# Mouafak-Khaled/Flow-Q-Learning

Hardware: AMD Instinct MI355X
Metric: FQL grad-steps/sec (whole node) over 16-α population, cube-single-v0 (higher is better)
Workload: dtype f32

## Files before the change

### flow-q-learning_amd/csrc/kernels.h

```cpp
#pragma once
#include <hip/hip_runtime.h>
#include <stdint.h>

namespace fq {

struct TRef {
    float* p;
    long long ss;
    long long sy;
};

inline TRef tref(float* p, long long ss, long long sy = 0) { return TRef{p, ss, sy}; }

enum GemmLayout { LAYOUT_FWD = 0, LAYOUT_DX = 1, LAYOUT_DW = 2 };
enum GemmEpi { EPI_STORE = 0, EPI_BIAS = 1, EPI_BIAS_GELU2 = 2, EPI_BIAS_GELU = 3, EPI_ADAM = 4 };

struct GemmArgs {
    TRef A, B, C, C2, bias;
    int M, N, K;
    int lda, ldb, ldc;
    int ny, nz;
    const int* slots;
    unsigned long long* probe;
};
// ... 87 lines not shown
};
void launch_head_fwd(int mode, const HeadArgs& a, hipStream_t s);

struct StreamArgs {
    const float* params;
    long long P, ens;
    long long w_off[EF_MAX_LAYERS + 1], b_off[EF_MAX_LAYERS + 1];
    long long g_off[EF_MAX_LAYERS], be_off[EF_MAX_LAYERS];
    const float* x0;
    long long x0_ss;
    int ld_x, K0, L, M;
    float* U[EF_MAX_LAYERS];
    float* G[EF_MAX_LAYERS];
    float* MU[EF_MAX_LAYERS];
    float* RS[EF_MAX_LAYERS];
    long long s_ss, s_sy, st_ss, st_sy;
    int ld_s, st_lo, st_hi;
    int g_hi;
    HeadArgs head;
    int ny, nz;
    const int* slots;
};
bool stream_fwd_supported(int H, int L, int K0, int nout, int M);
void launch_stream_fwd(int head_mode, bool ln, const StreamArgs& a, hipStream_t s);

struct SplitSync {
    unsigned long long* xch;
    unsigned* cnt;
    unsigned* gen;
    unsigned* err;
};
struct SplitFwdArgs {
    StreamArgs s;
    TRef aflow;
    int D, A, S, first;
    float steps_f;
    unsigned long long* probe;
    SplitSync sync;
    unsigned long long* phase;
    float* pre0;
};
long long split_cluster_bytes();
constexpr long long split_euler_pre0_floats() { return 2LL * 256 * 16; }
bool split_euler_pre0(int K0, int D);
int split_counter_stride();
bool split_fwd_supported(int H, int L, int K0, int nout, int M);
void launch_split_fwd(int head_mode, bool ln, bool euler, int F, const SplitFwdArgs& a, hipStream_t s);
// ... 273 lines not shown
```

### flow-q-learning_amd/csrc/kernels.hip

```cpp
#include "kernels.h"

#include <hip/hip_runtime.h>
#include <math.h>

#include <type_traits>

#if defined(__HIP_DEVICE_COMPILE__) && !defined(__gfx950__)
#error "fqlpop kernels target gfx950 (MI355X) only: the s_waitcnt immediates use the gfx9 encoding"
#endif


namespace fq {

typedef float f32x16 __attribute__((ext_vector_type(16)));
typedef float f32x4 __attribute__((ext_vector_type(4)));

#define DEV __device__ __forceinline__

DEV float* at(TRef t, int slot, int y = 0) {
    return t.p + (long long)slot * t.ss + (long long)y * t.sy;
}

constexpr float kSqrt2OverPi = 0.7978845608028654f;

// ... 161 lines not shown
        float* st = a.stats + ((long long)slot * a.n_total_chunks + ci) * 3;
        st[0] = mx;
        st[1] = mn;
        st[2] = ss;
    }
}
DEV void adam_chunk(const AdamArgs& a, int bx, int z) { adam_chunk_t<256>(a, bx, z); }



typedef __amdgpu_buffer_rsrc_t rsrc_t;
DEV rsrc_t make_rsrc(const float* p, long long n_elems) {
    return __builtin_amdgcn_make_buffer_rsrc((void*)p, (short)0, (int)(n_elems * 4), 0x00020000);
}
DEV float4 bload4(rsrc_t r, int elem_off) {
    return __builtin_bit_cast(float4, __builtin_amdgcn_raw_buffer_load_b128(r, elem_off * 4, 0, 0));
}
DEV float bload1(rsrc_t r, int voff_b, int soff_b) {
    return __builtin_bit_cast(float, __builtin_amdgcn_raw_buffer_load_b32(r, voff_b, soff_b, 0));
}
DEV void bstore1(rsrc_t r, float v, int voff_b, int soff_b) {
    __builtin_amdgcn_raw_buffer_store_b32(__builtin_bit_cast(int, v), r, voff_b, soff_b, 0);
}

template <int NT>
DEV void load_in0(float* in0, const float* x, int K0, int ld, int c0) {
    constexpr int N = 64 * 16 + 64, IT = (N + NT - 1) / NT;
    static_assert(N >= 16, "");
    const rsrc_t rX = make_rsrc(x, (long long)K0 * ld);
    float v[IT];
#pragma unroll
    for (int q = 0; q < IT; ++q) {
        const int e = min((int)threadIdx.x + q * NT, N - 1), r = e >> 4, j = e & 15;
        v[q] = bload1(rX, (r * ld + c0 + j) * 4, 0);
    }
#pragma unroll
    for (int q = 0; q < IT; ++q) {
        const int e = (int)threadIdx.x + q * NT;
        if (e < N) in0[e] = v[q];
    }
}

template <int TILE, int BK, bool RC>
DEV float4 stage_load(rsrc_t X, int ld, int p, int i0, int k0) {
    const int idx = threadIdx.x + 256 * p;
    if constexpr (RC) {
        const int row = idx / (BK / 4), c = (idx % (BK / 4)) * 4;
        return bload4(X, (i0 + row) * ld + k0 + c);
    } else {
        const int row = idx / (TILE / 4), c = (idx % (TILE / 4)) * 4;
        return bload4(X, (k0 + row) * ld + i0 + c);
    }
}

template <int BK, bool KB>
constexpr int rc_pitch() { return KB ? BK + 4 : BK + 1; }
// ... 1170 lines not shown
#pragma unroll
        for (int s = 0; s < 16; ++s) w5r[s] = li < nout ? w5r[s] : 0.f;
        f32x4 hacc = f32x4{0.f, 0.f, 0.f, 0.f};
#pragma unroll
        for (int s = 0; s < 16; ++s)
            hacc = __builtin_amdgcn_mfma_f32_16x16x4f32(w5r[s], slab[(64 * w + 4 * s + lk) * NC + li], hacc, 0, 0, 0);
        float* hred = in0;
        if (lk < 2) {
#pragma unroll
            for (int r = 0; r < 4; ++r) hred[w * 8 * NC + (4 * lk + r) * NC + li] = hacc[r];
        }
        __syncthreads();
        if (tid < nout * NC) {
            const int j = tid / NC, col = tid % NC;
            float v = hred[tid];
#pragma unroll
            for (int q = 1; q < EF_NW; ++q) v += hred[q * 8 * NC + tid];
            v += P[g.b_off[L] + j];
            head_write<MODE>(g.head, slot, y, j, c0 + col, v);
        }
    }
}

void launch_stream_fwd(int head_mode, bool ln, const StreamArgs& a, hipStream_t s) {
    const dim3 grid((a.M / EF_NC) * a.ny * a.nz), block(EF_NW * 64);
#define FQ_SF(MODE, LNV) hipLaunchKernelGGL((stream_fwd_kernel<MODE, LNV>), grid, block, 0, s, a)
    switch (head_mode) {
        case HEAD_BC_FUSED: if (ln) FQ_SF(HEAD_BC_FUSED, true); else FQ_SF(HEAD_BC_FUSED, false); break;
        case HEAD_OS: if (ln) FQ_SF(HEAD_OS, true); else FQ_SF(HEAD_OS, false); break;
        default: if (ln) FQ_SF(HEAD_STORE, true); else FQ_SF(HEAD_STORE, false); break;
    }
#undef FQ_SF
}

constexpr int SP_NW = 4, SP_NT = SP_NW * 64;
constexpr int SP_XG = EF_H * EF_NC;
constexpr int SP_G_HP = 2 * SP_XG;
constexpr int SP_G_LP = SP_G_HP + 8 * 8 * EF_NC;
constexpr int SP_G_N = SP_G_LP + 2 * 8 * 2 * EF_NC;
constexpr long long SP_CLUSTER_GRANULES = (SP_G_N + 31) / 32 * 32;
constexpr int SP_CNT_STRIDE = 16;
constexpr unsigned SP_SPIN_LIMIT = 1u << 21;

long long split_cluster_bytes() { return SP_CLUSTER_GRANULES * 8; }
int split_counter_stride() { return SP_CNT_STRIDE; }

typedef __attribute__((address_space(1))) unsigned int gu32_t;
typedef __attribute__((address_space(1))) unsigned long long gu64_t;

// ... 2708 lines not shown
```

### flow-q-learning_amd/csrc/runtime.cpp

```cpp
#include <hip/hip_runtime.h>

#include <algorithm>
#include <cmath>
#include <cstdio>
#include <cstdlib>
#include <cstring>
#include <functional>
#include <map>
#include <set>
#include <memory>
#include <string>
#include <vector>

#include "../../include/fqlpop.h"
#include "kernels.h"

using namespace fq;

namespace {

thread_local std::string g_err;

struct FqErr {
    int code;
// ... 16 lines not shown
long long align_up(long long x) { return (x + kAlign - 1) / kAlign * kAlign; }

#ifdef FQ_DIAG
const char* diag_env(const char* name) { return std::getenv(name); }
#else
const char* diag_env(const char*) { return nullptr; }
#endif

struct EngineOptions {
    int euler_fused = 1;
    int stream_fwd = 1;
    int stream_bwd = 1;
    int fused_adam = 1;
    int serial = 0;
    int dw_tile_critic = 10, dw_tile_actor = 10;
    int adam_nt = 3;
    int split = 1;
    int small_sched = 1;
    int split_blocks = 256;
    int split_sites = 0;
    int hw_queues = 4;
    int em_seq_sweep = 1;
    int em_ens_xcd = 0;
};
EngineOptions g_engine_opts;

constexpr int kStepBranches = 4;
int step_streams(const EngineOptions& eo) {
    return (eo.serial || eo.hw_queues < kStepBranches) ? 1 : kStepBranches;
}

struct EngineOptionRef {
    const char* name;
    int EngineOptions::*field;
    int lo, hi;
};
const EngineOptionRef kEngineOptions[] = {
    {"euler_fused", &EngineOptions::euler_fused, 0, 1}, {"stream_fwd", &EngineOptions::stream_fwd, 0, 1},
    {"stream_bwd", &EngineOptions::stream_bwd, 0, 1},   {"fused_adam", &EngineOptions::fused_adam, 0, 1},
    {"serial", &EngineOptions::serial, 0, 1},
    {"dw_tile_critic", &EngineOptions::dw_tile_critic, 0, 10},
    {"dw_tile_actor", &EngineOptions::dw_tile_actor, 0, 10},
    {"adam_nt", &EngineOptions::adam_nt, 0, 3},
    {"split", &EngineOptions::split, 0, 8},
    {"small_sched", &EngineOptions::small_sched, 0, 1},
    {"hw_queues", &EngineOptions::hw_queues, 1, 1024},
    {"split_sites", &EngineOptions::split_sites, 0, (1 << 24) - 1},
    {"split_blocks", &EngineOptions::split_blocks, 64, 1024},
    {"em_seq_sweep", &EngineOptions::em_seq_sweep, 0, 1},
    {"em_ens_xcd", &EngineOptions::em_ens_xcd, 0, 1},
};

void philox_host(uint32_t c[4], uint32_t k0, uint32_t k1) {
    for (int r = 0; r < 10; ++r) {
        const uint64_t p0 = (uint64_t)0xD2511F53u * c[0], p1 = (uint64_t)0xCD9E8D57u * c[2];
        const uint32_t hi0 = (uint32_t)(p0 >> 32), lo0 = (uint32_t)p0;
        const uint32_t hi1 = (uint32_t)(p1 >> 32), lo1 = (uint32_t)p1;
        const uint32_t n0 = hi1 ^ c[1] ^ k0, n2 = hi0 ^ c[3] ^ k1;
        c[0] = n0; c[1] = lo1; c[2] = n2; c[3] = lo0;
        k0 += 0x9E3779B9u;
        k1 += 0xBB67AE85u;
    }
}

uint64_t sample_key(uint64_t seed, float alpha) {
    uint32_t ab;
    std::memcpy(&ab, &alpha, sizeof(ab));
    uint64_t z = seed ^ ((uint64_t)ab << 32 | 0x9E3779B9u);
    z = (z ^ (z >> 30)) * 0xBF58476D1CE4E5B9ull;
    z = (z ^ (z >> 27)) * 0x94D049BB133111EBull;
    return z ^ (z >> 31);
}

// ... 54 lines not shown
    const Buf* X = nullptr;
    int ld = 0;
    int ld_d = 0, ld_o = 0;
    long long sy = 0, st_sy = 0;
    bool keep_u = true;
    bool dominant = false;
    std::vector<Buf> U, G, MU, RS, DU;
    Buf DH, C1, C2, part;
    int fwd_site = -1, bwd_site = -1;
    int skip_fwd = 0, skip_bwd = 0;
    TRef par(long long off) const { return tref(*arena + lay->off + off, arena_ss, lay->ens_size); }
    TRef act(const Buf& b, long long coff = 0) const { return b.cols(coff, sy); }
    TRef stat(const Buf& b, long long coff = 0) const { return b.cols(coff, st_sy); }
    TRef grad(const Buf& b) const { return b.ref((long long)lay->H * ld_d); }
};

}

struct fqlpop {
    fqlpop_config cfg{};
    EngineOptions opt{};
    int n = 0;
    int device = 0;
    int D = 0, A = 0, H = 0, L = 0, B = 0, E = 0, S = 0;
    NetLayout critic, bc, os;
    long long P = 0, PT = 0;
    std::vector<Leaf> leaves;
    long long state_size = 0;

    float* params_buf[2] = {nullptr, nullptr};
    Buf paramsT_buf[2];
    int cur = 0;
    float *params = nullptr, *params_nx = nullptr;
    float *grads = nullptr, *adam_m = nullptr, *adam_v = nullptr, *target = nullptr;
    int* count = nullptr;
    uint64_t* seeds = nullptr;
    uint64_t* skeys = nullptr;
    float* alpha = nullptr;
    int* slots = nullptr;
    float* stats = nullptr;
    Chunk* chunks = nullptr;
    int* chunk_leaf = nullptr;
    int* leaf_first = nullptr;
    int n_chunks_net[3] = {0, 0, 0}, chunk_base_net[3] = {0, 0, 0}, n_chunks_total = 0;
    bool fused_adam = false;
    int w_stat_base[3][EF_MAX_LAYERS] = {};
// ... 311 lines not shown
                                                                                        : kSplitMaxClusters;
}
constexpr long long kSplitMaxBlocks = 256;

int split_factor_opts(const EngineOptions& o, bool split_ok, int site, long long clusters, bool min4,
                      long long max_blocks) {
    int opt = o.split;
    const int code = (o.split_sites >> (3 * site)) & 7;
    if (code == 1) return 1;
    if (code >= 2 && code <= 4) {
        opt = 1 << (code - 1);
        max_blocks = std::max<long long>(max_blocks, clusters * opt);
    }
    if (!split_ok || opt == 0 || clusters > split_cap(site)) return 1;
    for (int F = std::max(opt >= 2 ? opt : 8, min4 ? 4 : 2); F >= 2; F /= 2) {
        if (min4 && F < 4) break;
        if (clusters * F <= max_blocks) return F;
    }
    return 1;
}
struct SplitShape {
    int H, L, A, B, E, K0bc, K0os, K0cr;
    bool critic_ln, stream_fwd, stream_bwd, fused_adam, euler_fused, multi_stream;
};
struct SplitPlan {
    int F[SITE_N];
    bool small;
};
SplitPlan split_plan(const EngineOptions& o, const SplitShape& d, int nz) {
    SplitPlan p{};
    int* F = p.F;
    const bool ok = d.stream_fwd && o.split != 0;
    const int B = d.B, B2 = 2 * B, B3 = 3 * B, T = B / 16;
    auto fwd = [&](int site, int K0, int nout, int M, long long clusters, bool min4) {
        F[site] = d.stream_fwd && split_fwd_supported(d.H, d.L, K0, nout, M)
                      ? split_factor_opts(o, ok, site, clusters, min4, o.split_blocks) : 1;
    };
    fwd(SITE_EULER, d.K0bc, d.A, B, (long long)T * nz, true);
    if (!d.euler_fused) F[SITE_EULER] = 1;
    p.small = o.small_sched && d.multi_stream && d.stream_fwd && d.stream_bwd && d.fused_adam &&
              (long long)T * nz <= kSmallSchedTiles;
    fwd(SITE_BCF, d.K0bc, d.A, B2, (long long)(B2 / 16) * nz, false);
    fwd(SITE_OSF, d.K0os, d.A, B3, (long long)(B3 / 16) * nz, false);
    fwd(SITE_TGT, d.K0cr, 1, B, (long long)T * d.E * nz, false);
    fwd(SITE_CRF, d.K0cr, 1, B2, (long long)(B2 / 16) * d.E * nz, false);
    auto bwd = [&](int site, int nout, int M, int Mg, long long clusters, bool min4) {
        F[site] = d.stream_bwd && split_bwd_supported(d.H, d.L, nout, M, Mg)
                      ? split_factor_opts(o, ok, site, clusters, min4, kSplitMaxBlocks) : 1;
    };
    if (p.small) {
        bwd(SITE_CRB, 1, B, 0, (long long)T * d.E * nz, d.critic_ln);
        bwd(SITE_CRB2, 1, B, B, (long long)T * d.E * nz, d.critic_ln);
    } else {
        bwd(SITE_CRB, 1, B2, B, (long long)(B2 / 16) * d.E * nz, d.critic_ln);
        F[SITE_CRB2] = 1;
    }
    bwd(SITE_OSB, d.A, B, B, (long long)T * nz, false);
    return p;
}
SplitPlan split_plan(const fqlpop* h, int nz) {
    const SplitShape d{h->H, h->L, h->A, h->B, h->E, h->bc.in_dim, h->os.in_dim, h->critic.in_dim, h->critic.ln,
                       h->stream_fwd, h->stream_bwd, h->fused_adam, h->euler_fused, h->sX != h->sM};
    return split_plan(h->opt, d, nz);
}

struct Ctx {
    fqlpop* h;
    int nz;
    SplitPlan plan;
};
Ctx step_ctx(fqlpop* h) { return Ctx{h, h->nz, split_plan(h, h->nz)}; }

SplitSync split_prep(fqlpop* h, int site, long long clusters, hipStream_t) {
    fqlpop::SplitSite& st = h->split_site[site];
    ARGCHK(clusters <= st.clusters, "split launch larger than its site");
    return SplitSync{st.xch, st.cnt, st.gen, h->split_err};
}

void fwd_hidden(const Ctx& c, hipStream_t s, const Net& n) {
    fqlpop* h = c.h;
    const NetLayout& N = *n.lay;
    for (int l = 0; l < N.L; ++l) {
        GemmArgs g{};
        g.A = n.par(N.W[l]);
        g.B = l == 0 ? n.X->ref() : n.act(n.G[l - 1]);
// ... 302 lines not shown
            a.U[l] = n.U[l].p;
            a.G[l] = n.G[l].p;
            if (stats && N.ln) { a.MU[l] = n.MU[l].p; a.RS[l] = n.RS[l].p; }
        }
    }
    a.x0 = n.X->p;
    a.x0_ss = n.X->ss;
    a.ld_x = n.ld; a.K0 = N.in_dim; a.L = N.L; a.M = n.ld;
    if (store) { a.s_ss = n.U[0].ss; a.s_sy = n.sy; }
    if (stats) { a.st_ss = n.MU[0].ss; a.st_sy = n.st_sy; }
    a.ld_s = n.ld; a.st_lo = k.st_lo; a.st_hi = k.st_hi;
    a.g_hi = k.g_hi < 0 ? k.st_hi : k.g_hi;
    a.head = head;
    a.head.nout = N.out_dim;
    a.ny = N.E; a.nz = c.nz; a.slots = h->slots;
    if (skip_mask() & n.skip_fwd) return;
    const int F = c.plan.F[n.fwd_site];
    if (F > 1) {
        SplitFwdArgs sa{};
        sa.s = a;
        sa.sync = split_prep(h, n.fwd_site, (long long)(n.ld / 16) * N.E * c.nz, s);
        launch_split_fwd(mode, N.ln, false, F, sa, s);
    } else {
        launch_stream_fwd(mode, N.ln, a, s);
    }
}

long long euler_blocks(const Ctx& c) { return (long long)(c.h->B / 16) * c.nz * c.plan.F[SITE_EULER]; }
SplitFwdArgs euler_split_args(const Ctx& c, const EulerArgs& ea, hipStream_t s) {
    fqlpop* h = c.h;
    const NetLayout& N = h->bc;
    SplitFwdArgs sa{};
    StreamArgs& a = sa.s;
    a.params = ea.params; a.P = ea.P; a.ens = 0;
    for (int l = 0; l <= N.L; ++l) { a.w_off[l] = ea.w_off[l]; a.b_off[l] = ea.b_off[l]; }
    a.x0 = ea.eu.p; a.x0_ss = ea.eu.ss; a.ld_x = ea.B; a.K0 = ea.D + ea.A + 1; a.L = ea.L; a.M = ea.B;
    a.head.nout = ea.A;
    a.ny = 1; a.nz = ea.nz; a.slots = ea.slots;
    sa.aflow = ea.aflow;
    sa.D = ea.D; sa.A = ea.A; sa.S = ea.S; sa.first = ea.first; sa.steps_f = ea.steps_f;
    sa.probe = ea.probe;
    sa.phase = ea.phase;
    sa.sync = split_prep(h, SITE_EULER, (long long)(ea.B / 16) * ea.nz, s);
    sa.pre0 = h->euler_pre0 && euler_blocks(c) <= h->euler_pre0_blocks ? h->euler_pre0 : nullptr;
    return sa;
}
void launch_euler(const Ctx& c, const EulerArgs& ea, hipStream_t s) {
// ... 557 lines not shown
                g_engine_opts.*o.field = value;
                return;
            }
        throw FqErr{FQLPOP_E_ARG, std::string("unknown engine option ") + name};
    });
}

int fqlpop_get_engine_option(const char* name, int* value) {
    return guard([&] {
        ARGCHK(name != nullptr && value != nullptr, "null argument");
        for (const EngineOptionRef& o : kEngineOptions)
            if (std::strcmp(o.name, name) == 0) {
                *value = g_engine_opts.*o.field;
                return;
            }
        throw FqErr{FQLPOP_E_ARG, std::string("unknown engine option ") + name};
    });
}

int fqlpop_reset_engine_options(void) {
    return guard([&] { g_engine_opts = EngineOptions{}; });
}

int fqlpop_split_plan(const fqlpop_config* cfg, int n_members, int* blocks_per_tile, int* small_sched) {
    return guard([&] {
        ARGCHK(cfg && blocks_per_tile && small_sched && n_members >= 1, "bad argument");
        const EngineOptions& eo = g_engine_opts;
        const int D = cfg->obs_dim, A = cfg->action_dim, B = cfg->batch_size, H = cfg->hidden_dim, L = cfg->num_hidden;
        SplitShape d{H, L, A, B, cfg->num_qs, D + A + 1, D + A, D + A, cfg->layer_norm != 0,
                     stream_fwd_supported(H, L, D + A + 1, A, B) && eo.stream_fwd != 0,
                     stream_bwd_supported(H, L, A, B, B) && eo.stream_bwd != 0, false,
                     euler_flow_supported(H, L, D, A, B) && !cfg->actor_layer_norm && eo.euler_fused != 0,
                     step_streams(eo) > 1};
        d.fused_adam = d.stream_bwd && H % 128 == 0 && L <= GEMM_GROUP_MAX && eo.fused_adam;
        const SplitPlan p = split_plan(eo, d, n_members);
        for (int i = 0; i < SITE_N; ++i) blocks_per_tile[i] = p.F[i];
        *small_sched = p.small ? 1 : 0;
    });
}

int fqlpop_step_streams(int* n_streams) {
    return guard([&] {
        ARGCHK(n_streams != nullptr, "null argument");
        *n_streams = step_streams(g_engine_opts);
    });
}

int fqlpop_diagnostic_build(void) {
#ifdef FQ_DIAG
    return 1;
#else
    return 0;
#endif
}

double fqlpop_flops_per_member_step(const fqlpop_config* c) {
    const double B = c->batch_size, H = c->hidden_dim, L = c->num_hidden, D = c->obs_dim, A = c->action_dim;
    const double E = c->num_qs, S = c->flow_steps;
    auto F = [&](double i, double o) { return 2.0 * B * (i * H + (L - 1) * H * H + H * o); };
    auto dX = [&](double o) { return 2.0 * B * ((L - 1) * H * H + H * o); };
// ... 5 lines not shown
int fqlpop_create(const fqlpop_config* cfg, int n_members, const float* alphas, const uint64_t* seeds_in,
                  int device, fqlpop_t** out) {
    return guard([&] {
        ARGCHK(cfg && out && alphas && seeds_in, "null argument");
        ARGCHK(n_members > 0, "n_members must be > 0");
        ARGCHK(cfg->action_dim >= 1 && cfg->action_dim <= 8, "action_dim must be in [1, 8]");
        ARGCHK(cfg->obs_dim >= 1, "obs_dim must be >= 1");
        {
            const int hd = cfg->hidden_dim;
            ARGCHK(hd == 64 || hd == 128 || hd == 256 || hd == 512 || hd == 1024,
                   "hidden_dim must be one of 64, 128, 256, 512, 1024");
        }
        ARGCHK(cfg->num_hidden >= 1, "num_hidden must be >= 1");
        ARGCHK(cfg->batch_size >= 64 && cfg->batch_size % 64 == 0, "batch_size must be a multiple of 64");
        ARGCHK(cfg->num_qs >= 1 && cfg->num_qs <= 4, "num_qs must be in [1, 4]");
        ARGCHK(cfg->flow_steps >= 2, "flow_steps must be >= 2");
        if (cfg->actor_layer_norm)
            throw FqErr{FQLPOP_E_UNSUPPORTED, "actor_layer_norm is not supported yet (reference default False)"};
        auto h = std::make_unique<fqlpop>();
        h->cfg = *cfg;
        h->n = n_members;
        h->device = device;
        HIPCHK(hipSetDevice(device));
        h->D = cfg->obs_dim; h->A = cfg->action_dim; h->H = cfg->hidden_dim; h->L = cfg->num_hidden;
        h->B = cfg->batch_size; h->E = cfg->num_qs; h->S = cfg->flow_steps;
        const int D = h->D, A = h->A, H = h->H, L = h->L, B = h->B, E = h->E;
        h->critic.build("critic", D + A, 1, L, H, E, cfg->layer_norm != 0);
        h->bc.build("actor_bc_flow", D + A + 1, A, L, H, 1, cfg->actor_layer_norm != 0);
        h->os.build("actor_onestep_flow", D + A, A, L, H, 1, cfg->actor_layer_norm != 0);
        h->critic.off = 0;
        h->bc.off = align_up(h->critic.size());
        h->os.off = align_up(h->bc.off + h->bc.size());
        h->P = align_up(h->os.off + h->os.size());
        h->PT = align_up(h->critic.size());
        build_leaves(h.get());

        h->opt = g_engine_opts;
        const EngineOptions& eo = h->opt;
        HIPCHK(hipStreamCreateWithFlags(&h->sM, hipStreamNonBlocking));
        if (step_streams(eo) == 1) {
            h->sF = h->sB = h->sX = h->sM;
        } else {
            HIPCHK(hipStreamCreateWithFlags(&h->sF, hipStreamNonBlocking));
            HIPCHK(hipStreamCreateWithFlags(&h->sB, hipStreamNonBlocking));
            HIPCHK(hipStreamCreateWithFlags(&h->sX, hipStreamNonBlocking));
        }
// ... 1365 lines not shown
```

### flow-q-learning_amd/fqlpop/_lib.py

```python
from __future__ import annotations

import ctypes
import os

try:
    import torch
except Exception:
    torch = None

_HERE = os.path.dirname(os.path.abspath(__file__))
LIB_PATH = os.path.join(_HERE, "libfqlpop.so")

INFO_STRIDE = 16
TRAIN_INFO_KEYS = (
    "critic/critic_loss", "critic/q_mean", "critic/q_max", "critic/q_min",
    "actor/actor_loss", "actor/bc_flow_loss", "actor/distill_loss",
    "actor/q_loss", "actor/q", "actor/mse",
    "grad/max", "grad/min", "grad/norm",
)
VAL_INFO_KEYS = TRAIN_INFO_KEYS[:10]
STATE_PARAMS, STATE_ADAM_M, STATE_ADAM_V = 0, 1, 2


class FqlpopError(RuntimeError):
# ... 43 lines not shown
        ("init_lr", ctypes.c_float), ("reconstruction_weight", ctypes.c_float),
        ("seed", ctypes.c_uint64),
    ]


EM_STATE_PREDICTOR, EM_TERMINATION, EM_MULTISTEP = 0, 1, 2
ENS_PER_MODEL, ENS_MIXED = 0, 1
ENS_MAX_MODELS = 16
EM_LOG_STRIDE = 8
INITOBS_LOG_STRIDE = 4
INITOBS_LOG_KEYS = ("reconstruction_loss", "kl", "loss")
_P = ctypes.c_void_p
_F = ctypes.POINTER(ctypes.c_float)
_U8 = ctypes.POINTER(ctypes.c_uint8)
_SIGS = {
    "fqlpop_last_error": (ctypes.c_char_p, []),
    "fqlpop_set_engine_option": (ctypes.c_int, [ctypes.c_char_p, ctypes.c_int]),
    "fqlpop_get_engine_option": (ctypes.c_int, [ctypes.c_char_p, ctypes.POINTER(ctypes.c_int)]),
    "fqlpop_reset_engine_options": (ctypes.c_int, []),
    "fqlpop_diagnostic_build": (ctypes.c_int, []),
    "fqlpop_step_streams": (ctypes.c_int, [ctypes.POINTER(ctypes.c_int)]),
    "fqlpop_split_plan": (ctypes.c_int, [ctypes.c_void_p, ctypes.c_int, ctypes.POINTER(ctypes.c_int),
                                         ctypes.POINTER(ctypes.c_int)]),
    "fqlpop_probe_coverage": (ctypes.c_int, [ctypes.c_void_p, ctypes.POINTER(ctypes.c_int64),
                                             ctypes.POINTER(ctypes.c_int64)]),
    "fqlpop_create": (ctypes.c_int, [ctypes.POINTER(Config), ctypes.c_int, _F,
                                     ctypes.POINTER(ctypes.c_uint64), ctypes.c_int,
                                     ctypes.POINTER(_P)]),
    "fqlpop_destroy": (ctypes.c_int, [_P]),
    "fqlpop_set_dataset": (ctypes.c_int, [_P, ctypes.c_int, _P, _P, _P, _P, _P,
                                          ctypes.c_int64, ctypes.c_int]),
    "fqlpop_set_active": (ctypes.c_int, [_P, ctypes.POINTER(ctypes.c_uint8)]),
    "fqlpop_step": (ctypes.c_int, [_P, ctypes.c_int]),
    "fqlpop_step_injected": (ctypes.c_int, [_P, _F, _F]),
    "fqlpop_total_loss": (ctypes.c_int, [_P, _F, _F]),
    "fqlpop_read_info": (ctypes.c_int, [_P, ctypes.c_int, _F]),
    "fqlpop_sample_actions": (ctypes.c_int, [_P, ctypes.c_int, _F, ctypes.c_int64, _F,
                                             ctypes.c_uint64, _F]),
    "fqlpop_state_size": (ctypes.c_int, [_P, ctypes.POINTER(ctypes.c_int64)]),
    "fqlpop_get_state": (ctypes.c_int, [_P, ctypes.c_int, ctypes.c_int, _F, ctypes.c_int64]),
    "fqlpop_set_state": (ctypes.c_int, [_P, ctypes.c_int, ctypes.c_int, _F, ctypes.c_int64]),
    "fqlpop_get_count": (ctypes.c_int, [_P, ctypes.c_int, ctypes.POINTER(ctypes.c_int32)]),
    "fqlpop_set_count": (ctypes.c_int, [_P, ctypes.c_int, ctypes.c_int32]),
    "fqlpop_set_member": (ctypes.c_int, [_P, ctypes.c_int, ctypes.c_float, ctypes.c_uint64,
                                         ctypes.c_int]),
    "fqlpop_clone_members": (ctypes.c_int, [_P, ctypes.c_int, ctypes.POINTER(ctypes.c_int),
# ... 157 lines not shown
```

### flow-q-learning_amd/fqlpop/population.py

```python
from __future__ import annotations

import ctypes
from dataclasses import dataclass

import numpy as np

from fqlpop import _lib
from fqlpop._lib import (INFO_STRIDE, STATE_ADAM_M, STATE_ADAM_V, STATE_PARAMS,
                         TRAIN_INFO_KEYS, VAL_INFO_KEYS, check, fptr)


@dataclass
class PopulationConfig:
    obs_dim: int = 28
    action_dim: int = 5
    hidden_dims: tuple = (512, 512, 512, 512)
    batch_size: int = 256
    num_qs: int = 2
    layer_norm: bool = True
    actor_layer_norm: bool = False
    flow_steps: int = 10
    q_agg: str = "mean"
    normalize_q_loss: bool = False
    discount: float = 0.99
# ... 21 lines not shown
        if tuple(cfg.get("actor_hidden_dims", (512,) * 4)) != tuple(cfg.get("value_hidden_dims", (512,) * 4)):
            raise ValueError("actor_hidden_dims must equal value_hidden_dims")
        if cfg.get("encoder") not in (None, "None"):
            raise ValueError("visual encoders are out of scope (encoder must be None)")
        return cls(obs_dim=obs_dim, action_dim=action_dim,
                   hidden_dims=tuple(cfg.get("value_hidden_dims", (512,) * 4)),
                   batch_size=int(cfg.get("batch_size", 256)),
                   layer_norm=bool(cfg.get("layer_norm", True)),
                   actor_layer_norm=bool(cfg.get("actor_layer_norm", False)),
                   flow_steps=int(cfg.get("flow_steps", 10)), q_agg=cfg.get("q_agg", "mean"),
                   normalize_q_loss=bool(cfg.get("normalize_q_loss", False)),
                   discount=float(cfg.get("discount", 0.99)), tau=float(cfg.get("tau", 0.005)),
                   lr=float(cfg.get("lr", 3e-4)), **kw)


def _f32(a) -> np.ndarray:
    return np.ascontiguousarray(np.asarray(a, dtype=np.float32))


SPLIT_SITES = ("bc_forward", "euler_flow", "onestep_forward", "target_critic", "critic_forward", "critic_backward",
               "onestep_backward", "critic_backward_td")


def split_plan(cfg: "PopulationConfig", n_members: int) -> dict:
    c = cfg.to_c()
    F = (ctypes.c_int * 8)()
    small = ctypes.c_int()
    check(_lib.load_library().fqlpop_split_plan(ctypes.byref(c), int(n_members), F, ctypes.byref(small)))
    out = dict(zip(SPLIT_SITES, [int(x) for x in F]))
    out["small_sched"] = bool(small.value)
    return out


class Population:

    def __init__(self, cfg: PopulationConfig, alphas, seeds, device: int = 0):
        self.lib = _lib.load_library()
        self.cfg = cfg
        alphas = _f32(alphas).reshape(-1)
        seeds = np.ascontiguousarray(np.asarray(seeds, dtype=np.uint64).reshape(-1))
        if alphas.shape != seeds.shape:
            raise ValueError("alphas and seeds must have the same length")
        self.n = int(alphas.shape[0])
        self.alphas = alphas.copy()
        self.seeds = seeds.copy()
        self._c = cfg.to_c()
        hwq = _lib.hw_queues_from_env()
        prev_hwq = _lib.get_engine_option("hw_queues") if hwq is not None else None
        if hwq is not None:
            _lib.set_engine_option("hw_queues", hwq)
        h = ctypes.c_void_p()
        try:
            check(self.lib.fqlpop_create(ctypes.byref(self._c), self.n, fptr(alphas),
# ... 460 lines not shown
```

### include/fqlpop.h

```cpp
#ifndef FQLPOP_H
#define FQLPOP_H

#include <stddef.h>
#include <stdint.h>

#ifdef __cplusplus
extern "C" {
#endif

#define FQLPOP_OK 0
#define FQLPOP_E_ARG (-1)
#define FQLPOP_E_HIP (-2)
#define FQLPOP_E_STATE (-3)
#define FQLPOP_E_UNSUPPORTED (-4)

#define FQLPOP_INFO_STRIDE 16
enum {
    FQLPOP_INFO_CRITIC_LOSS = 0, FQLPOP_INFO_Q_MEAN, FQLPOP_INFO_Q_MAX, FQLPOP_INFO_Q_MIN,
    FQLPOP_INFO_ACTOR_LOSS, FQLPOP_INFO_BC_FLOW_LOSS, FQLPOP_INFO_DISTILL_LOSS,
    FQLPOP_INFO_Q_LOSS, FQLPOP_INFO_Q, FQLPOP_INFO_MSE,
    FQLPOP_INFO_GRAD_MAX, FQLPOP_INFO_GRAD_MIN, FQLPOP_INFO_GRAD_NORM
};

enum { FQLPOP_STATE_PARAMS = 0, FQLPOP_STATE_ADAM_M = 1, FQLPOP_STATE_ADAM_V = 2 };
// ... 4 lines not shown
    int hidden_dim;
    int num_hidden;
    int batch_size;
    int num_qs;
    int layer_norm;
    int actor_layer_norm;
    int flow_steps;
    int q_agg_min;
    int normalize_q_loss;
    float discount;
    float tau;
    float lr;
    int use_graph;
} fqlpop_config;

typedef struct fqlpop fqlpop_t;

const char* fqlpop_last_error(void);

int fqlpop_set_engine_option(const char* name, int value);
int fqlpop_get_engine_option(const char* name, int* value);
int fqlpop_reset_engine_options(void);
int fqlpop_split_plan(const fqlpop_config* cfg, int n_members, int* blocks_per_tile, int* small_sched);
int fqlpop_step_streams(int* n_streams);
int fqlpop_diagnostic_build(void);

int fqlpop_create(const fqlpop_config* cfg, int n_members, const float* alphas,
                  const uint64_t* seeds, int device, fqlpop_t** out);

int fqlpop_destroy(fqlpop_t* h);

int fqlpop_set_dataset(fqlpop_t* h, int which, const float* obs, const float* act,
                       const float* rew, const float* mask, const float* next_obs,
                       int64_t n_rows, int on_device);

int fqlpop_set_active(fqlpop_t* h, const uint8_t* mask);

int fqlpop_step(fqlpop_t* h, int n_steps);

int fqlpop_step_injected(fqlpop_t* h, const float* batch, const float* noise);

int fqlpop_total_loss(fqlpop_t* h, const float* batch, const float* noise);

int fqlpop_read_info(fqlpop_t* h, int which, float* out);

int fqlpop_sample_actions(fqlpop_t* h, int member, const float* obs, int64_t n,
// ... 185 lines not shown
```

Baseline: 8457.

## Add 32-column streaming forward kernel reusing each weight load across two column tiles

Adds a stream_fwd2 kernel in which each block handles 32 batch columns instead of 16. Every weight float4 loaded from the ring feeds two MFMAs, one per 16-column half, which halves weight traffic per column. Stores are widened to float2. A per-site planner picks 32 columns for the critic, one-step and BC forward sites only when column ranges are aligned and the grid still has at least one block per CU. The price is half as many blocks, more accumulator registers and doubled shared memory per block, which can hurt occupancy and latency hiding.

```diff
diff --git a/flow-q-learning_amd/csrc/kernels.h b/flow-q-learning_amd/csrc/kernels.h
--- a/flow-q-learning_amd/csrc/kernels.h
+++ b/flow-q-learning_amd/csrc/kernels.h
@@ -133,7 +133,7 @@
     const int* slots;
 };
 bool stream_fwd_supported(int H, int L, int K0, int nout, int M);
-void launch_stream_fwd(int head_mode, bool ln, const StreamArgs& a, hipStream_t s);
+void launch_stream_fwd(int head_mode, bool ln, const StreamArgs& a, hipStream_t s, int cols = 16);
 
 struct SplitSync {
     unsigned long long* xch;
diff --git a/flow-q-learning_amd/csrc/kernels.hip b/flow-q-learning_amd/csrc/kernels.hip
--- a/flow-q-learning_amd/csrc/kernels.hip
+++ b/flow-q-learning_amd/csrc/kernels.hip
@@ -207,16 +207,20 @@
 DEV void bstore1(rsrc_t r, float v, int voff_b, int soff_b) {
     __builtin_amdgcn_raw_buffer_store_b32(__builtin_bit_cast(int, v), r, voff_b, soff_b, 0);
 }
-
-template <int NT>
+typedef unsigned int u32x2 __attribute__((ext_vector_type(2)));
+DEV void bstore2(rsrc_t r, float2 v, int voff_b, int soff_b) {
+    __builtin_amdgcn_raw_buffer_store_b64(__builtin_bit_cast(u32x2, v), r, voff_b, soff_b, 0);
+}
+
+template <int NT, int NCOL = 16>
 DEV void load_in0(float* in0, const float* x, int K0, int ld, int c0) {
-    constexpr int N = 64 * 16 + 64, IT = (N + NT - 1) / NT;
-    static_assert(N >= 16, "");
+    constexpr int N = 64 * NCOL + 4 * NCOL, IT = (N + NT - 1) / NT;
+    static_assert(NCOL == 16 || NCOL == 32, "");
     const rsrc_t rX = make_rsrc(x, (long long)K0 * ld);
     float v[IT];
 #pragma unroll
     for (int q = 0; q < IT; ++q) {
-        const int e = min((int)threadIdx.x + q * NT, N - 1), r = e >> 4, j = e & 15;
+        const int e = min((int)threadIdx.x + q * NT, N - 1), r = e / NCOL, j = e % NCOL;
         v[q] = bload1(rX, (r * ld + c0 + j) * 4, 0);
     }
 #pragma unroll
@@ -1433,9 +1437,229 @@
     }
 }
 
-void launch_stream_fwd(int head_mode, bool ln, const StreamArgs& a, hipStream_t s) {
-    const dim3 grid((a.M / EF_NC) * a.ny * a.nz), block(EF_NW * 64);
-#define FQ_SF(MODE, LNV) hipLaunchKernelGGL((stream_fwd_kernel<MODE, LNV>), grid, block, 0, s, a)
+constexpr int EF_NC2 = 2 * EF_NC;
+
+DEV void ef_kloop2(f32x4 (&acc)[2][4], float4 (&ring)[EF_PF], rsrc_t rW, const float* xs, int NS, int w_cur,
+                   int w_next, int lo, int lk, int li) {
+    constexpr int H = EF_H, PF = EF_PF;
+    const float2* xs2 = reinterpret_cast<const float2*>(xs);
+    float2 bnext = xs2[lk * EF_NC + li];
+    int s0 = 0;
+    do {
+        const int rbase = (s0 + PF < NS ? w_cur + 4 * (s0 + PF) * H : w_next) + lo;
+#pragma unroll
+        for (int p = 0; p < PF; ++p) {
+            const int s = s0 + p;
+            const float2 b = bnext;
+            bnext = xs2[(4 * (s + 1) + lk) * EF_NC + li];
+            __builtin_amdgcn_sched_barrier(0);
+            const float4 a = ring[p];
+            acc[0][0] = __builtin_amdgcn_mfma_f32_16x16x4f32(a.x, b.x, acc[0][0], 0, 0, 0);
+            acc[1][0] = __builtin_amdgcn_mfma_f32_16x16x4f32(a.x, b.y, acc[1][0], 0, 0, 0);
+            acc[0][1] = __builtin_amdgcn_mfma_f32_16x16x4f32(a.y, b.x, acc[0][1], 0, 0, 0);
+            acc[1][1] = __builtin_amdgcn_mfma_f32_16x16x4f32(a.y, b.y, acc[1][1], 0, 0, 0);
+            acc[0][2] = __builtin_amdgcn_mfma_f32_16x16x4f32(a.z, b.x, acc[0][2], 0, 0, 0);
+            acc[1][2] = __builtin_amdgcn_mfma_f32_16x16x4f32(a.z, b.y, acc[1][2], 0, 0, 0);
+            acc[0][3] = __builtin_amdgcn_mfma_f32_16x16x4f32(a.w, b.x, acc[0][3], 0, 0, 0);
+            acc[1][3] = __builtin_amdgcn_mfma_f32_16x16x4f32(a.w, b.y, acc[1][3], 0, 0, 0);
+            __builtin_amdgcn_sched_barrier(0);
+            ring[p] = bload4(rW, rbase + 4 * p * H);
+            __builtin_amdgcn_sched_barrier(0);
+        }
+        s0 += PF;
+    } while (s0 < NS);
+}
+
+template <int MODE, bool LN>
+__global__ __launch_bounds__(EF_NW * 64, 1) void stream_fwd2_kernel(const StreamArgs g) {
+    constexpr int H = EF_H, NC = EF_NC2, NT = EF_NW * 64, PF = EF_PF;
+    __shared__ __attribute__((aligned(16))) float slab[H * NC + 4 * NC];
+    __shared__ __attribute__((aligned(16))) float in0[EF_K0MAX * NC + 4 * NC];
+    __shared__ float lnred[2][EF_NW][NC];
+    __shared__ float lnp[3][H];
+
+    const int tiles = g.M / NC;
+    const int total = tiles * g.ny * g.nz;
+    const int bid = xcd_remap(blockIdx.x, total);
+    const int tile = bid % tiles, yz = bid / tiles;
+    const int y = yz % g.ny, z = yz / g.ny;
+    const int slot = g.slots[z];
+    const int c0 = tile * NC;
+    const int tid = threadIdx.x, lane = tid & 63;
+    const int w = __builtin_amdgcn_readfirstlane(tid >> 6);
+    const int li = lane & 15, lk = lane >> 4;
+    const int L = g.L, K0 = g.K0, nout = g.head.nout;
+    const bool tail0 = K0 > 4 * PF && K0 <= 4 * (PF + 1);
+    const int NS0 = tail0 ? PF : (K0 + 4 * PF - 1) / (4 * PF) * PF;
+    const float* __restrict__ P = g.params + (long long)slot * g.P + (long long)y * g.ens;
+    const float* __restrict__ x0 = g.x0 + (long long)slot * g.x0_ss;
+    load_in0<NT, NC>(in0, x0, K0, g.ld_x, c0);
+    const rsrc_t rW = make_rsrc(P, g.P);
+    const int lo = lk * H + 64 * w + 4 * li;
+    float4 ring[PF];
+#pragma unroll
+    for (int p = 0; p < PF; ++p) ring[p] = bload4(rW, (int)g.w_off[0] + 4 * p * H + lo);
+    const bool st = c0 >= g.st_lo && c0 + NC <= g.st_hi;
+    const int m = c0 + 2 * li;
+    if constexpr (LN) {
+        lnp[0][tid] = P[g.b_off[0] + tid];
+        lnp[1][tid] = P[g.g_off[0] + tid];
+        lnp[2][tid] = P[g.be_off[0] + tid];
+    }
+    __syncthreads();
+
+    for (int l = 0; l < L; ++l) {
+        const int NS = l == 0 ? NS0 : H / 4;
+        const float* xs = l == 0 ? in0 : slab;
+        const int nl = l + 1 < L ? l + 1 : 0;
+        f32x4 acc[2][4];
+#pragma unroll
+        for (int t = 0; t < 2; ++t)
+#pragma unroll
+            for (int c = 0; c < 4; ++c) acc[t][c] = f32x4{0.f, 0.f, 0.f, 0.f};
+        const int lp = LN ? nl : l;
+        const float pb = P[g.b_off[lp] + tid];
+        const float pg = LN ? P[g.g_off[lp] + tid] : 0.f;
+        const float pe = LN ? P[g.be_off[lp] + tid] : 0.f;
+        const int wcur = (int)g.w_off[l], wnext = (int)g.w_off[nl];
+        asm volatile("" ::"s"(wcur), "s"(wnext));
+        const float4 at0 = bload4(rW, wcur + 4 * PF * H + lo);
+        ef_kloop2(acc, ring, rW, xs, NS, wcur, wnext, lo, lk, li);
+        if (l == 0 && tail0) {
+            const float2 b = reinterpret_cast<const float2*>(xs)[(4 * PF + lk) * EF_NC + li];
+            const float av[4] = {at0.x, at0.y, at0.z, at0.w};
+#pragma unroll
+            for (int c = 0; c < 4; ++c) {
+                acc[0][c] = __builtin_amdgcn_mfma_f32_16x16x4f32(av[c], b.x, acc[0][c], 0, 0, 0);
+                acc[1][c] = __builtin_amdgcn_mfma_f32_16x16x4f32(av[c], b.y, acc[1][c], 0, 0, 0);
+            }
+        }
+        if constexpr (!LN) {
+            lnp[0][tid] = pb;
+            __syncthreads();
+        }
+
+        const bool stU = st && g.U[l];
+        const bool stGb = st && g.G[l] && c0 < g.g_hi;
+        const bool stG = stGb && m + 2 <= g.g_hi;
+        const long long sbase = (long long)slot * g.s_ss + (long long)y * g.s_sy + c0;
+        const rsrc_t rU = make_rsrc(stU ? g.U[l] + sbase : g.params, stU ? (long long)H * g.ld_s : 0);
+        const rsrc_t rG = make_rsrc(stGb ? g.G[l] + sbase : g.params, stGb ? (long long)H * g.ld_s : 0);
+        const int svo = ((64 * w + 16 * lk) * g.ld_s + 2 * li) * 4;
+        float v[2][4][4];
+#pragma unroll
+        for (int r = 0; r < 4; ++r) {
+            const float4 bb = *reinterpret_cast<const float4*>(&lnp[0][64 * w + 16 * lk + 4 * r]);
+            const float bv[4] = {bb.x, bb.y, bb.z, bb.w};
+#pragma unroll
+            for (int c = 0; c < 4; ++c) {
+                const float u0 = acc[0][c][r] + bv[c], u1 = acc[1][c][r] + bv[c];
+                if (stU) bstore2(rU, float2{u0, u1}, svo, (4 * r + c) * g.ld_s * 4);
+                v[0][r][c] = gelu_fast(u0);
+                v[1][r][c] = gelu_fast(u1);
+            }
+        }
+        if constexpr (LN) {
+            float mean[2], rs[2];
+            float s1[2] = {0.f, 0.f}, s2[2] = {0.f, 0.f};
+#pragma unroll
+            for (int t = 0; t < 2; ++t) {
+#pragma unroll
+                for (int r = 0; r < 4; ++r)
+#pragma unroll
+                    for (int c = 0; c < 4; ++c) ln_acc(v[t][r][c], s1[t], s2[t]);
+                s1[t] = lk_sum(s1[t]);
+                s2[t] = lk_sum(s2[t]);
+            }
+            if (lk == 0) {
+                *reinterpret_cast<float2*>(&lnred[0][w][2 * li]) = float2{s1[0], s1[1]};
+                *reinterpret_cast<float2*>(&lnred[1][w][2 * li]) = float2{s2[0], s2[1]};
+            }
+            __syncthreads();
+            lnp[0][tid] = pb;
+            float S1[2] = {0.f, 0.f}, S2[2] = {0.f, 0.f};
+#pragma unroll
+            for (int q = 0; q < EF_NW; ++q) {
+                const float2 a1 = *reinterpret_cast<const float2*>(&lnred[0][q][2 * li]);
+                const float2 a2 = *reinterpret_cast<const float2*>(&lnred[1][q][2 * li]);
+                S1[0] += a1.x; S1[1] += a1.y;
+                S2[0] += a2.x; S2[1] += a2.y;
+            }
+#pragma unroll
+            for (int t = 0; t < 2; ++t) ln_stats(S1[t], S2[t], (float)H, mean[t], rs[t]);
+#pragma unroll
+            for (int r = 0; r < 4; ++r) {
+                const float4 g4 = *reinterpret_cast<const float4*>(&lnp[1][64 * w + 16 * lk + 4 * r]);
+                const float4 b4 = *reinterpret_cast<const float4*>(&lnp[2][64 * w + 16 * lk + 4 * r]);
+                const float ga[4] = {g4.x, g4.y, g4.z, g4.w};
+                const float be[4] = {b4.x, b4.y, b4.z, b4.w};
+#pragma unroll
+                for (int t = 0; t < 2; ++t)
+#pragma unroll
+                    for (int c = 0; c < 4; ++c) v[t][r][c] = ln_apply(v[t][r][c], mean[t], rs[t], ga[c], be[c]);
+            }
+            if (st && w == 0 && lk == 0 && g.MU[l]) {
+                const long long so = (long long)slot * g.st_ss + (long long)y * g.st_sy + m;
+#pragma unroll
+                for (int t = 0; t < 2; ++t) {
+                    g.MU[l][so + t] = mean[t];
+                    g.RS[l][so + t] = rs[t];
+                }
+            }
+        }
+#pragma unroll
+        for (int r = 0; r < 4; ++r)
+#pragma unroll
+            for (int c = 0; c < 4; ++c) {
+                const int f = 64 * w + 16 * lk + 4 * r + c;
+                const float2 o = float2{v[0][r][c], v[1][r][c]};
+                if (stG) bstore2(rG, o, svo, (4 * r + c) * g.ld_s * 4);
+                *reinterpret_cast<float2*>(&slab[f * NC + 2 * li]) = o;
+            }
+        __syncthreads();
+        if constexpr (LN) {
+            lnp[1][tid] = pg;
+            lnp[2][tid] = pe;
+        }
+    }
+    {
+        float w5r[16];
+#pragma unroll
+        for (int s = 0; s < 16; ++s) w5r[s] = bload1(rW, ((int)g.w_off[L] + (64 * w + 4 * s + lk) * nout + li) * 4, 0);
+#pragma unroll
+        for (int s = 0; s < 16; ++s) w5r[s] = li < nout ? w5r[s] : 0.f;
+        f32x4 hacc[2] = {f32x4{0.f, 0.f, 0.f, 0.f}, f32x4{0.f, 0.f, 0.f, 0.f}};
+#pragma unroll
+        for (int s = 0; s < 16; ++s) {
+            const float2 b = *reinterpret_cast<const float2*>(&slab[(64 * w + 4 * s + lk) * NC + 2 * li]);
+            hacc[0] = __builtin_amdgcn_mfma_f32_16x16x4f32(w5r[s], b.x, hacc[0], 0, 0, 0);
+            hacc[1] = __builtin_amdgcn_mfma_f32_16x16x4f32(w5r[s], b.y, hacc[1], 0, 0, 0);
+        }
+        float* hred = in0;
+        if (lk < 2) {
+#pragma unroll
+            for (int r = 0; r < 4; ++r)
+                *reinterpret_cast<float2*>(&hred[w * 8 * NC + (4 * lk + r) * NC + 2 * li]) = float2{hacc[0][r], hacc[1][r]};
+        }
+        __syncthreads();
+        if (tid < nout * NC) {
+            const int j = tid / NC, col = tid % NC;
+            float v = hred[tid];
+#pragma unroll
+            for (int q = 1; q < EF_NW; ++q) v += hred[q * 8 * NC + tid];
+            v += P[g.b_off[L] + j];
+            head_write<MODE>(g.head, slot, y, j, c0 + col, v);
+        }
+    }
+}
+
+void launch_stream_fwd(int head_mode, bool ln, const StreamArgs& a, hipStream_t s, int cols) {
+    const dim3 grid((a.M / cols) * a.ny * a.nz), block(EF_NW * 64);
+#define FQ_SF(MODE, LNV)                                                                             \
+    do {                                                                                             \
+        if (cols == EF_NC2) hipLaunchKernelGGL((stream_fwd2_kernel<MODE, LNV>), grid, block, 0, s, a); \
+        else hipLaunchKernelGGL((stream_fwd_kernel<MODE, LNV>), grid, block, 0, s, a);               \
+    } while (0)
     switch (head_mode) {
         case HEAD_BC_FUSED: if (ln) FQ_SF(HEAD_BC_FUSED, true); else FQ_SF(HEAD_BC_FUSED, false); break;
         case HEAD_OS: if (ln) FQ_SF(HEAD_OS, true); else FQ_SF(HEAD_OS, false); break;
diff --git a/flow-q-learning_amd/csrc/runtime.cpp b/flow-q-learning_amd/csrc/runtime.cpp
--- a/flow-q-learning_amd/csrc/runtime.cpp
+++ b/flow-q-learning_amd/csrc/runtime.cpp
@@ -62,8 +62,10 @@
     int hw_queues = 4;
     int em_seq_sweep = 1;
     int em_ens_xcd = 0;
+    int fwd_cols32 = 7;
 };
 EngineOptions g_engine_opts;
+constexpr int kDefaultCus = 256;
 
 constexpr int kStepBranches = 4;
 int step_streams(const EngineOptions& eo) {
@@ -89,6 +91,7 @@
     {"split_blocks", &EngineOptions::split_blocks, 64, 1024},
     {"em_seq_sweep", &EngineOptions::em_seq_sweep, 0, 1},
     {"em_ens_xcd", &EngineOptions::em_ens_xcd, 0, 1},
+    {"fwd_cols32", &EngineOptions::fwd_cols32, 0, 15},
 };
 
 void philox_host(uint32_t c[4], uint32_t k0, uint32_t k1) {
@@ -189,6 +192,7 @@
     EngineOptions opt{};
     int n = 0;
     int device = 0;
+    int n_cus = kDefaultCus;
     int D = 0, A = 0, H = 0, L = 0, B = 0, E = 0, S = 0;
     NetLayout critic, bc, os;
     long long P = 0, PT = 0;
@@ -546,11 +550,27 @@
 struct SplitShape {
     int H, L, A, B, E, K0bc, K0os, K0cr;
     bool critic_ln, stream_fwd, stream_bwd, fused_adam, euler_fused, multi_stream;
+    int n_cus = kDefaultCus;
 };
 struct SplitPlan {
     int F[SITE_N];
     bool small;
+    int cols[SITE_N];
 };
+
+constexpr int kColsBitCritic = 1, kColsBitOs = 2, kColsBitBc = 4, kColsBitAnyBlocks = 8;
+int fwd_cols_rule(const EngineOptions& o, int site, int F, int M, int E, int nz, int st_lo, int st_hi, int g_hi,
+                  int col_off, int n_cus) {
+    const int bit = site == SITE_TGT || site == SITE_CRF ? kColsBitCritic
+                    : site == SITE_OSF                   ? kColsBitOs
+                    : site == SITE_BCF                   ? kColsBitBc
+                                                         : 0;
+    if (!(o.fwd_cols32 & bit) || F != 1) return 16;
+    if (M % 32 || st_lo % 32 || st_hi % 32 || col_off % 32 || g_hi % 2) return 16;
+    if (!(o.fwd_cols32 & kColsBitAnyBlocks) && (long long)(M / 32) * E * nz < n_cus) return 16;
+    return 32;
+}
+
 SplitPlan split_plan(const EngineOptions& o, const SplitShape& d, int nz) {
     SplitPlan p{};
     int* F = p.F;
@@ -580,11 +600,21 @@
         F[SITE_CRB2] = 1;
     }
     bwd(SITE_OSB, d.A, B, B, (long long)T * nz, false);
+    for (int& c : p.cols) c = 16;
+    if (d.stream_fwd) {
+        auto cols = [&](int site, int M, int E, int st_lo, int st_hi, int g_hi) {
+            p.cols[site] = fwd_cols_rule(o, site, F[site], M, E, nz, st_lo, st_hi, g_hi, 0, d.n_cus);
+        };
+        cols(SITE_BCF, B2, 1, 0, B, B);
+        cols(SITE_OSF, B3, 1, B, B2, B2);
+        cols(SITE_TGT, B, d.E, 0, 0, 0);
+        cols(SITE_CRF, B2, d.E, 0, B2, d.stream_bwd ? B : B2);
+    }
     return p;
 }
 SplitPlan split_plan(const fqlpop* h, int nz) {
     const SplitShape d{h->H, h->L, h->A, h->B, h->E, h->bc.in_dim, h->os.in_dim, h->critic.in_dim, h->critic.ln,
-                       h->stream_fwd, h->stream_bwd, h->fused_adam, h->euler_fused, h->sX != h->sM};
+                       h->stream_fwd, h->stream_bwd, h->fused_adam, h->euler_fused, h->sX != h->sM, h->n_cus};
     return split_plan(h->opt, d, nz);
 }
 
@@ -933,7 +963,10 @@
         sa.sync = split_prep(h, n.fwd_site, (long long)(n.ld / 16) * N.E * c.nz, s);
         launch_split_fwd(mode, N.ln, false, F, sa, s);
     } else {
-        launch_stream_fwd(mode, N.ln, a, s);
+        const int cols = c.plan.cols[n.fwd_site];
+        ARGCHK(cols == 16 || (cols == 32 && a.M % 32 == 0 && a.st_lo % 32 == 0 && a.st_hi % 32 == 0 && a.g_hi % 2 == 0),
+               "32-column forward planned for a launch whose column ranges do not allow it");
+        launch_stream_fwd(mode, N.ln, a, s, cols);
     }
 }
 
@@ -1537,20 +1570,36 @@
     return guard([&] { g_engine_opts = EngineOptions{}; });
 }
 
+}
+namespace {
+SplitPlan config_plan(const fqlpop_config* cfg, int n_members, int n_cus) {
+    const EngineOptions& eo = g_engine_opts;
+    const int D = cfg->obs_dim, A = cfg->action_dim, B = cfg->batch_size, H = cfg->hidden_dim, L = cfg->num_hidden;
+    SplitShape d{H, L, A, B, cfg->num_qs, D + A + 1, D + A, D + A, cfg->layer_norm != 0,
+                 stream_fwd_supported(H, L, D + A + 1, A, B) && eo.stream_fwd != 0,
+                 stream_bwd_supported(H, L, A, B, B) && eo.stream_bwd != 0, false,
+                 euler_flow_supported(H, L, D, A, B) && !cfg->actor_layer_norm && eo.euler_fused != 0,
+                 step_streams(eo) > 1, n_cus};
+    d.fused_adam = d.stream_bwd && H % 128 == 0 && L <= GEMM_GROUP_MAX && eo.fused_adam;
+    return split_plan(eo, d, n_members);
+}
+}
+extern "C" {
+
 int fqlpop_split_plan(const fqlpop_config* cfg, int n_members, int* blocks_per_tile, int* small_sched) {
     return guard([&] {
         ARGCHK(cfg && blocks_per_tile && small_sched && n_members >= 1, "bad argument");
-        const EngineOptions& eo = g_engine_opts;
-        const int D = cfg->obs_dim, A = cfg->action_dim, B = cfg->batch_size, H = cfg->hidden_dim, L = cfg->num_hidden;
-        SplitShape d{H, L, A, B, cfg->num_qs, D + A + 1, D + A, D + A, cfg->layer_norm != 0,
-                     stream_fwd_supported(H, L, D + A + 1, A, B) && eo.stream_fwd != 0,
-                     stream_bwd_supported(H, L, A, B, B) && eo.stream_bwd != 0, false,
-                     euler_flow_supported(H, L, D, A, B) && !cfg->actor_layer_norm && eo.euler_fused != 0,
-                     step_streams(eo) > 1};
-        d.fused_adam = d.stream_bwd && H % 128 == 0 && L <= GEMM_GROUP_MAX && eo.fused_adam;
-        const SplitPlan p = split_plan(eo, d, n_members);
+        const SplitPlan p = config_plan(cfg, n_members, kDefaultCus);
         for (int i = 0; i < SITE_N; ++i) blocks_per_tile[i] = p.F[i];
         *small_sched = p.small ? 1 : 0;
+    });
+}
+
+int fqlpop_fwd_cols_plan(const fqlpop_config* cfg, int n_members, int n_cus, int* cols_per_block) {
+    return guard([&] {
+        ARGCHK(cfg && cols_per_block && n_members >= 1 && n_cus >= 1, "bad argument");
+        const SplitPlan p = config_plan(cfg, n_members, n_cus);
+        for (int i = 0; i < SITE_N; ++i) cols_per_block[i] = p.cols[i];
     });
 }
 
@@ -1602,6 +1651,7 @@
         h->n = n_members;
         h->device = device;
         HIPCHK(hipSetDevice(device));
+        HIPCHK(hipDeviceGetAttribute(&h->n_cus, hipDeviceAttributeMultiprocessorCount, device));
         h->D = cfg->obs_dim; h->A = cfg->action_dim; h->H = cfg->hidden_dim; h->L = cfg->num_hidden;
         h->B = cfg->batch_size; h->E = cfg->num_qs; h->S = cfg->flow_steps;
         const int D = h->D, A = h->A, H = h->H, L = h->L, B = h->B, E = h->E;
diff --git a/flow-q-learning_amd/fqlpop/_lib.py b/flow-q-learning_amd/fqlpop/_lib.py
--- a/flow-q-learning_amd/fqlpop/_lib.py
+++ b/flow-q-learning_amd/fqlpop/_lib.py
@@ -89,6 +89,7 @@
     "fqlpop_step_streams": (ctypes.c_int, [ctypes.POINTER(ctypes.c_int)]),
     "fqlpop_split_plan": (ctypes.c_int, [ctypes.c_void_p, ctypes.c_int, ctypes.POINTER(ctypes.c_int),
                                          ctypes.POINTER(ctypes.c_int)]),
+    "fqlpop_fwd_cols_plan": (ctypes.c_int, [ctypes.c_void_p, ctypes.c_int, ctypes.c_int, ctypes.POINTER(ctypes.c_int)]),
     "fqlpop_probe_coverage": (ctypes.c_int, [ctypes.c_void_p, ctypes.POINTER(ctypes.c_int64),
                                              ctypes.POINTER(ctypes.c_int64)]),
     "fqlpop_create": (ctypes.c_int, [ctypes.POINTER(Config), ctypes.c_int, _F,
diff --git a/flow-q-learning_amd/fqlpop/population.py b/flow-q-learning_amd/fqlpop/population.py
--- a/flow-q-learning_amd/fqlpop/population.py
+++ b/flow-q-learning_amd/fqlpop/population.py
@@ -67,13 +67,20 @@
                "onestep_backward", "critic_backward_td")
 
 
-def split_plan(cfg: "PopulationConfig", n_members: int) -> dict:
+FWD_SITES = ("bc_forward", "onestep_forward", "target_critic", "critic_forward")
+
+
+def split_plan(cfg: "PopulationConfig", n_members: int, n_cus: int = 256) -> dict:
     c = cfg.to_c()
     F = (ctypes.c_int * 8)()
     small = ctypes.c_int()
     check(_lib.load_library().fqlpop_split_plan(ctypes.byref(c), int(n_members), F, ctypes.byref(small)))
     out = dict(zip(SPLIT_SITES, [int(x) for x in F]))
     out["small_sched"] = bool(small.value)
+    cols = (ctypes.c_int * 8)()
+    check(_lib.load_library().fqlpop_fwd_cols_plan(ctypes.byref(c), int(n_members), int(n_cus), cols))
+    by_site = dict(zip(SPLIT_SITES, [int(x) for x in cols]))
+    out["fwd_cols"] = {s: by_site[s] for s in FWD_SITES}
     return out
 
 
diff --git a/include/fqlpop.h b/include/fqlpop.h
--- a/include/fqlpop.h
+++ b/include/fqlpop.h
@@ -50,6 +50,7 @@
 int fqlpop_get_engine_option(const char* name, int* value);
 int fqlpop_reset_engine_options(void);
 int fqlpop_split_plan(const fqlpop_config* cfg, int n_members, int* blocks_per_tile, int* small_sched);
+int fqlpop_fwd_cols_plan(const fqlpop_config* cfg, int n_members, int n_cus, int* cols_per_block);
 int fqlpop_step_streams(int* n_streams);
 int fqlpop_diagnostic_build(void);
 
```

New measurement: 8539 (median of 6 runs). About the same (+1.0%).
